# ultralytics/yolov5

Measured on NVIDIA H100. Metric: images/sec @640 (forward + NMS), higher is better.
Workload: dtype bf16

## Files before the change

### include/y5b200.h

```cpp
#ifndef Y5B200_H
#define Y5B200_H
#include <stdint.h>

#if defined(__GNUC__)
#define Y5_API __attribute__((visibility("default")))
#else
#define Y5_API
#endif

#ifdef __cplusplus
extern "C" {
#endif

#define Y5_F16 0
#define Y5_BF16 1
#define Y5_F32 2
#define Y5_U8 3

#define Y5_E_INVALID (-1)
#define Y5_E_UNSUPPORTED (-2)
#define Y5_E_DRIVER (-3)

#define Y5_ACT_NONE 0
#define Y5_ACT_SILU 1
// ... 25 lines not shown
    int64_t in_n_stride;
    int32_t a_mode;
    int32_t reserved;
} y5_conv_desc;

int y5_conv_pick(int32_t in_c, int32_t out_c, int64_t m_rows, int32_t* block_k, int32_t* block_n);

typedef struct y5_conv_plan y5_conv_plan;
int y5_conv_plan_create(const y5_conv_desc* desc, y5_conv_plan** plan);
int y5_conv_plan_run(const y5_conv_plan* plan, void* stream);
void y5_conv_plan_destroy(y5_conv_plan* plan);
struct y5_conv_plan_info {
    int32_t a_mode;
    int32_t tw, th;
    int32_t block_k, block_n, mt;
    int32_t cluster;
    int32_t patch_pw;
    int32_t b_grouped;
    int32_t staged;
    int32_t opt;
    int32_t epi;
    int32_t a_stages, b_stages;
    int32_t grid;
};
int y5_conv_plan_info(const y5_conv_plan* plan, struct y5_conv_plan_info* info);
int y5_conv_bn_silu_fwd(const y5_conv_desc* desc, void* stream);
int y5_conv_direct_fwd(const y5_conv_desc* desc, void* stream);

typedef struct y5_detect_desc {
    const void* in;
    int32_t in_pitch;
    int32_t batch, ny, nx, in_c;
    const void* weight;
    const float* bias;
    void* raw;
    void* z;
    int32_t z_rows, z_row0;
    int32_t na, no, nc;
    float stride;
    float anchor_wh[8];
    int32_t dtype;
    int32_t block_k;
} y5_detect_desc;
typedef struct y5_detect_plan y5_detect_plan;
int y5_detect_plan_create(const y5_detect_desc* desc, y5_detect_plan** plan);
int y5_detect_plan_run(const y5_detect_plan* plan, void* stream);
// ... 305 lines not shown
```

### yolov5_b200/_lib.py

```python
from __future__ import annotations

import ctypes as C
import os

import torch

_HERE = os.path.dirname(os.path.abspath(__file__))
LIB_PATH = os.environ.get("Y5B200_LIB") or os.path.join(_HERE, "liby5b200.so")

Y5_F16, Y5_BF16, Y5_F32, Y5_U8 = 0, 1, 2, 3
ACT_NONE, ACT_SILU = 0, 1

_DTYPE = {torch.float16: Y5_F16, torch.bfloat16: Y5_BF16, torch.float32: Y5_F32, torch.uint8: Y5_U8}


def dtype_code(dt: torch.dtype) -> int:
    try:
        return _DTYPE[dt]
    except KeyError:
        raise TypeError(f"y5b200: unsupported dtype {dt}") from None


class ConvDesc(C.Structure):
    _fields_ = [
# ... 9 lines not shown
        ("a_mode", C.c_int32), ("reserved", C.c_int32),
    ]


class DetectDesc(C.Structure):
    _fields_ = [
        ("inp", C.c_void_p), ("in_pitch", C.c_int32),
        ("batch", C.c_int32), ("ny", C.c_int32), ("nx", C.c_int32), ("in_c", C.c_int32),
        ("weight", C.c_void_p), ("bias", C.c_void_p),
        ("raw", C.c_void_p), ("z", C.c_void_p),
        ("z_rows", C.c_int32), ("z_row0", C.c_int32),
        ("na", C.c_int32), ("no", C.c_int32), ("nc", C.c_int32),
        ("stride", C.c_float), ("anchor_wh", C.c_float * 8),
        ("dtype", C.c_int32), ("block_k", C.c_int32),
    ]


class PlanInfo(C.Structure):
    _fields_ = [
        ("a_mode", C.c_int32), ("tw", C.c_int32), ("th", C.c_int32),
        ("block_k", C.c_int32), ("block_n", C.c_int32), ("mt", C.c_int32), ("cluster", C.c_int32),
        ("patch_pw", C.c_int32), ("b_grouped", C.c_int32), ("staged", C.c_int32), ("opt", C.c_int32), ("epi", C.c_int32),
        ("a_stages", C.c_int32), ("b_stages", C.c_int32), ("grid", C.c_int32),
    ]

    def as_dict(self) -> dict:
        return {f: getattr(self, f) for f, _ in self._fields_}


class NmsParams(C.Structure):
    _fields_ = [
        ("batch", C.c_int32), ("n_rows", C.c_int32), ("no", C.c_int32), ("nc", C.c_int32), ("nm", C.c_int32),
        ("dtype", C.c_int32), ("conf_thres", C.c_float), ("iou_thres", C.c_float),
        ("multi_label", C.c_int32), ("agnostic", C.c_int32), ("max_det", C.c_int32), ("max_nms", C.c_int32),
        ("max_wh", C.c_float), ("classes", C.c_void_p), ("n_classes", C.c_int32),
    ]


class LossParams(C.Structure):
    _fields_ = [
        ("nl", C.c_int32), ("batch", C.c_int32), ("na", C.c_int32), ("no", C.c_int32), ("nc", C.c_int32),
        ("ny", C.c_int32 * 5), ("nx", C.c_int32 * 5),
        ("dtype", C.c_int32), ("nt", C.c_int32),
        ("anchor_t", C.c_float), ("box_gain", C.c_float), ("obj_gain", C.c_float), ("cls_gain", C.c_float),
        ("cls_pw", C.c_float), ("obj_pw", C.c_float), ("cp", C.c_float), ("cn", C.c_float),
        ("balance", C.c_float * 5), ("grad_scale", C.c_float),
# ... 213 lines not shown
```

### yolov5_b200/csrc/common.cuh

```cuda
#pragma once
#include <cuda.h>
#include <cuda_bf16.h>
#include <cuda_fp16.h>
#include <cuda_runtime.h>
#include <stdint.h>
#include <stdio.h>

namespace y5 {

__device__ __forceinline__ uint32_t smem_u32(const void* p) { return static_cast<uint32_t>(__cvta_generic_to_shared(p)); }

__device__ __forceinline__ bool elect_one() {
    uint32_t pred = 0;
    asm volatile(
        "{\n\t.reg .pred P;\n\t"
        "elect.sync _|P, 0xffffffff;\n\t"
        "selp.b32 %0, 1, 0, P;\n\t}"
        : "=r"(pred));
    return pred != 0;
}

__device__ __forceinline__ void mbar_init(uint64_t* bar, uint32_t count) {
    asm volatile("mbarrier.init.shared::cta.b64 [%0], %1;" ::"r"(smem_u32(bar)), "r"(count) : "memory");
}
// ... 105 lines not shown
    return (((8u * row_bytes) >> 4) & 0x3FFFu) | (layout << 30);
}
__device__ __forceinline__ uint32_t gmma_desc_lo(uint32_t saddr) { return ((saddr >> 4) & 0x3FFFu) | (1u << 16); }
__device__ __forceinline__ uint64_t gmma_desc(uint32_t lo, uint32_t hi) { return (static_cast<uint64_t>(hi) << 32) | lo; }

__device__ __forceinline__ void wgmma_fence() { asm volatile("wgmma.fence.sync.aligned;" ::: "memory"); }
__device__ __forceinline__ void wgmma_commit() { asm volatile("wgmma.commit_group.sync.aligned;" ::: "memory"); }
template <int N>
__device__ __forceinline__ void wgmma_wait() { asm volatile("wgmma.wait_group.sync.aligned %0;" ::"n"(N) : "memory"); }
template <int N>
__device__ __forceinline__ void fence_regs(float (&d)[N]) {
#pragma unroll
    for (int i = 0; i < N; ++i) asm volatile("" : "+f"(d[i])::"memory");
}

template <uint32_t R>
__device__ __forceinline__ void setmaxnreg_dec() { asm volatile("setmaxnreg.dec.sync.aligned.u32 %0;" ::"n"(R)); }
template <uint32_t R>
__device__ __forceinline__ void setmaxnreg_inc() { asm volatile("setmaxnreg.inc.sync.aligned.u32 %0;" ::"n"(R)); }

__device__ __forceinline__ void griddep_wait() { asm volatile("griddepcontrol.wait;" ::: "memory"); }
__device__ __forceinline__ void griddep_launch_dependents() { asm volatile("griddepcontrol.launch_dependents;" ::: "memory"); }

__device__ __forceinline__ void named_bar_sync(uint32_t id, uint32_t nthreads) {
    asm volatile("bar.sync %0, %1;" ::"r"(id), "r"(nthreads) : "memory");
}

#ifndef Y5_SILU_EXACT
__device__ __forceinline__ float silu_f(float x) {
    const float h = 0.5f * x;
    float t;
    asm("tanh.approx.f32 %0, %1;" : "=f"(t) : "f"(h));
    return fmaf(h, t, h);
}
__device__ __forceinline__ float silu_from_half(float h) {
    float t;
    asm("tanh.approx.f32 %0, %1;" : "=f"(t) : "f"(h));
    return fmaf(h, t, h);
}
#else
__device__ __forceinline__ float silu_f(float x) { return __fdividef(x, 1.0f + __expf(-x)); }
__device__ __forceinline__ float silu_from_half(float h) { return silu_f(2.0f * h); }
#endif
__device__ __forceinline__ float silu_tail(float x) {
    float e;
    asm("ex2.approx.f32 %0, %1;" : "=f"(e) : "f"(1.44269504088896341f * x));
// ... 31 lines not shown
```

### yolov5_b200/csrc/conv_gemm.cu

```cuda
#include <cstdio>
#include <cstdlib>
#include <cstring>
#include <mutex>
#include <type_traits>

#include "../../include/y5b200.h"
#include "common.cuh"
#include "host_util.h"
#include "wgmma.cuh"

namespace y5 {

constexpr int kBlockM = 128;
constexpr int kConsumers = 2;
constexpr int kConsumerThreads = 128 * kConsumers;
constexpr int kThreads = 128 + kConsumerThreads;
constexpr int kMaxStages = 8;
constexpr int kHeadN = 128;

enum AMode { A_LINEAR = 0, A_IM2COL = 1, A_PATCH = 2 };

struct ConvParams {
    int M, N;
    int num_m_tiles;
    int num_m_super, num_n_tiles;
    int kh, kw, c_chunks;
    int block_k;
    int a_mode;
    int Ho, Wo, HoWo, stride, pad_h, pad_w;
    int tw, th, tiles_x, tiles_y;
    int b_grouped;
    int patch_pw;
    int cluster_n;
    uint32_t stg_bytes;
    uint32_t b_sub_bytes;
    float rcp_per_img, rcp_tiles_x, rcp_HoWo, rcp_Wo;
    int a_stages, b_stages;
    uint32_t a_sub_bytes, a_stage_bytes, b_stage_bytes;
    int is_bf16, act;
    const float* bias;
    int bias_n;
    void* out;
    int out_pitch;
    const void* res;
    int res_pitch;
    void* raw;
    void* z;
    int na, no, nc, nx, z_rows, z_row0;
    float det_stride;
    float anchor_wh[8];
};

struct SmemLayout {
    uint32_t off_a, off_b, off_out, off_bias, off_bars, total;
};

__host__ __device__ inline SmemLayout smem_layout(int epi, int no, int bias_n, int a_stages, int b_stages, uint32_t a_bytes,
                                                   uint32_t b_bytes, uint32_t stg_bytes) {
    SmemLayout L;
    uint32_t o = 0;
    L.off_a = o;
    o += a_stages * a_bytes;
    L.off_b = o;
    o += b_stages * b_bytes;
    o = (o + 1023) & ~1023u;
    L.off_out = o;
    if (epi == 1) o += 4 * ((kBlockM * no * 2 + 1023) & ~1023u);
    else o += stg_bytes;
    L.off_bias = o;
    o += ((bias_n + 3) & ~3) * 4;
    o = (o + 7) & ~7u;
    L.off_bars = o;
    o += 4 * kMaxStages * 8;
    L.total = o;
    return L;
}

__device__ __forceinline__ int fdiv(int n, int d, float rd) {
    if (n >= (1 << 23)) return n / d;
    int q = __float2int_rz(__int2float_rz(n) * rd);
    const int r = n - q * d;
    if (r >= d) ++q;
    else if (r < 0) --q;
    return q;
}

template <int BLOCK_N, int MT, int KS, bool BF16>
__device__ __forceinline__ void mma_batch(float (&acc)[MT][BLOCK_N / 2], uint32_t a_lo, uint32_t a_sub16, uint32_t a_hi, uint32_t b_lo,
                                          uint32_t b_hi, uint32_t scale_first) {
    wgmma_fence();
#pragma unroll
    for (int k = 0; k < KS; ++k)
#pragma unroll
        for (int mi = 0; mi < MT; ++mi)
            Wgmma<BLOCK_N>::template run<BF16, 0, 0>(acc[mi], gmma_desc(a_lo + mi * a_sub16 + 2 * k, a_hi), gmma_desc(b_lo + 2 * k, b_hi),
                                                     k == 0 ? scale_first : 1u);
    wgmma_commit();
}

template <int BLOCK_N, int EPI, int MT, bool OPT, bool BF16>
__global__ void __launch_bounds__(kThreads, 1)
conv_gemm_kernel(const __grid_constant__ CUtensorMap tmA, const __grid_constant__ CUtensorMap tmB, const ConvParams p) {
    static_assert(MT * BLOCK_N <= 256, "accumulators: at most 128 fp32 registers per consumer thread");
    constexpr int kAcc = BLOCK_N / 2;

    extern __shared__ __align__(1024) uint8_t smem_raw[];
    uint8_t* smem = reinterpret_cast<uint8_t*>((reinterpret_cast<uintptr_t>(smem_raw) + 1023) & ~uintptr_t(1023));
    const SmemLayout L = smem_layout(EPI, p.no, p.bias_n, p.a_stages, p.b_stages, p.a_stage_bytes, p.b_stage_bytes, p.stg_bytes);
    uint8_t* sA = smem + L.off_a;
    uint8_t* sB = smem + L.off_b;
    float* sBias = reinterpret_cast<float*>(smem + L.off_bias);
    uint64_t* a_full = reinterpret_cast<uint64_t*>(smem + L.off_bars);
    uint64_t* a_empty = a_full + kMaxStages;
    uint64_t* b_full = a_empty + kMaxStages;
    uint64_t* b_empty = b_full + kMaxStages;

    const int warp = threadIdx.x >> 5;
    const int lane = threadIdx.x & 31;
    const int csize = OPT ? static_cast<int>(cluster_nctarank()) : 1;
    const uint32_t crank = OPT ? cluster_ctarank() : 0u;

    if (threadIdx.x == 0) {
        tma_prefetch_desc(&tmA);
        tma_prefetch_desc(&tmB);
        for (int s = 0; s < kMaxStages; ++s) {
            mbar_init(&a_full[s], 1);
            mbar_init(&a_empty[s], kConsumers);
            mbar_init(&b_full[s], 1);
            mbar_init(&b_empty[s], kConsumers * csize);
        }
        fence_barrier_init();
    }
    if (threadIdx.x >= 128)
        for (int i = threadIdx.x - 128; i < p.bias_n; i += kConsumerThreads) {
            const float b = i < p.N ? __ldg(p.bias + i) : 0.0f;
            sBias[i] = (EPI == 0 && p.act) ? 0.5f * b : b;
        }
    __syncthreads();
    if (csize > 1) cluster_sync_all();
    griddep_wait();
    griddep_launch_dependents();

    const int nn = p.num_n_tiles;
    const int num_tiles = ((p.num_m_super + csize - 1) / csize) * nn;
    const int tile0 = blockIdx.x / csize, tile_step = gridDim.x / csize;
    const uint32_t row_bytes = p.block_k * 2;
    const bool patch = p.a_mode == A_PATCH;
    const bool wide = OPT && p.patch_pw > 0;
    const int grp = wide ? p.kh * p.kw : (patch ? p.kh : 1);
    const int num_groups = wide ? p.c_chunks : (patch ? p.c_chunks * p.kw : p.kh * p.kw * p.c_chunks);

    if (warp < 4) {
        setmaxnreg_dec<56>();
    }
    if (warp == 0) {
        int as = 0, bs = 0;
        uint32_t aph = 0, bph = 0;
        for (int tile = tile0; tile < num_tiles; tile += tile_step) {
            const int ms = (tile / nn) * csize + static_cast<int>(crank);
            const int n0 = (tile - (tile / nn) * nn) * BLOCK_N;
            int img[MT], y0[MT], x0[MT];
#pragma unroll
            for (int mi = 0; mi < MT; ++mi) {
                const int mt = ms * MT + mi;
                img[mi] = y0[mi] = x0[mi] = 0;
                if (p.a_mode == A_IM2COL) {
                    const int m0 = mt * kBlockM;
                    img[mi] = fdiv(m0, p.HoWo, p.rcp_HoWo);
                    const int rem = m0 - img[mi] * p.HoWo;
                    const int oy = fdiv(rem, p.Wo, p.rcp_Wo);
                    y0[mi] = oy * p.stride - p.pad_h;
                    x0[mi] = (rem - oy * p.Wo) * p.stride - p.pad_w;
                } else if (patch) {
                    const int per_img = p.tiles_x * p.tiles_y;
                    img[mi] = fdiv(mt, per_img, p.rcp_per_img);
                    const int rem = mt - img[mi] * per_img;
                    const int ty = fdiv(rem, p.tiles_x, p.rcp_tiles_x);
                    y0[mi] = ty * p.th - p.pad_h;
                    x0[mi] = (rem - ty * p.tiles_x) * p.tw - p.pad_w;
                }
// ... 25 lines not shown
                        if (stage_first) mbar_arrive_expect_tx(&b_full[bs], p.b_stage_bytes);
                        uint8_t* b_dst = sB + bs * p.b_stage_bytes + (p.b_grouped ? j * p.b_sub_bytes : 0u);
                        if (csize == 1) tma_load_2d(&tmB, &b_full[bs], b_dst, kb * p.block_k, n0);
                        else {
                            const int slice_rows = BLOCK_N / csize;
                            tma_load_2d_mcast(&tmB, &b_full[bs], b_dst + crank * slice_rows * row_bytes, kb * p.block_k,
                                              n0 + static_cast<int>(crank) * slice_rows, static_cast<uint16_t>((1u << csize) - 1u));
                        }
                    }
                    __syncwarp();
                    if (stage_last && ++bs == p.b_stages) { bs = 0; bph ^= 1; }
                }
            };
            if (wide) {
                for (int cc = 0; cc < p.c_chunks; ++cc) issue_group(cc, 0, 0);
            } else if (patch) {
                for (int cc = 0; cc < p.c_chunks; ++cc)
                    for (int s = 0; s < p.kw; ++s) issue_group(cc, s, 0);
            } else {
                for (int r = 0; r < p.kh; ++r)
                    for (int s = 0; s < p.kw; ++s)
                        for (int cc = 0; cc < p.c_chunks; ++cc) issue_group(cc, s, r);
            }
        }
    } else if (warp >= 4) {
    setmaxnreg_inc<224>();
    const int wg = (warp >> 2) - 1;
    const int ct = threadIdx.x - 128;
    const int wrow = wg * 64 + (warp & 3) * 16 + (lane >> 2);
    const int ccol = 2 * (lane & 3);
    const bool signal = (threadIdx.x & 127) == 0;
    constexpr bool bf16 = BF16;
    const uint32_t dhi = gmma_desc_hi(row_bytes);
    const uint32_t a_hi = wide ? (dhi & ~0x3FFFu) | (((static_cast<uint32_t>(p.patch_pw) * row_bytes) >> 4) & 0x3FFFu) : dhi;
    const uint32_t a_base = gmma_desc_lo(smem_u32(sA) + (wide ? wg * 8 * p.patch_pw : wg * 64) * row_bytes), b_base = gmma_desc_lo(smem_u32(sB));
    const uint32_t row16 = row_bytes >> 4;
    const uint32_t a_stage16 = p.a_stage_bytes >> 4, b_stage16 = p.b_stage_bytes >> 4, a_sub16 = p.a_sub_bytes >> 4;
    const uint32_t b_sub16 = p.b_sub_bytes >> 4;
    const uint32_t a_shift16 = patch ? (p.tw * row_bytes) >> 4 : 0;
    const int k_steps = p.block_k / 16;
    const int per_img = p.tiles_x * p.tiles_y;
    const int tw_shift = patch ? __ffs(p.tw) - 1 : 0;
    int as = 0, bs = 0, head_set = 0;
    uint32_t aph = 0, bph = 0;
    float acc[MT][kAcc];
#pragma unroll
    for (int mi = 0; mi < MT; ++mi)
#pragma unroll
        for (int i = 0; i < kAcc; ++i) acc[mi][i] = 0.0f;

    int pend_as = 0, pend_bs = 0;
    bool pend_a_last = false, pend_b_last = false;
    auto release_pending = [&]() {
        if (!signal) return;
        if (pend_b_last) {
            if (csize == 1) mbar_arrive(&b_empty[pend_bs]);
            else
                for (int r = 0; r < csize; ++r) mbar_arrive_cluster(mapa_u32(&b_empty[pend_bs], static_cast<uint32_t>(r)));
        }
        if (pend_a_last) mbar_arrive(&a_empty[pend_as]);
    };

    for (int tile = tile0; tile < num_tiles; tile += tile_step) {
        const int ms = (tile / nn) * csize + static_cast<int>(crank);
        const int nt = tile - (tile / nn) * nn;
        const int n0 = nt * BLOCK_N;
        for (int g = 0; g < num_groups; ++g) {
            mbar_wait(&a_full[as], aph);
            const uint32_t a_stage_lo = a_base + as * a_stage16;
            uint32_t a_lo = a_stage_lo;
            for (int j = 0; j < grp; ++j) {
                if (wide) {
                    const int tr = j / p.kw, ts = j - tr * p.kw;
                    a_lo = a_stage_lo + (tr * p.patch_pw + ts) * row16;
                }
                const bool stage_first = !p.b_grouped || j == 0, stage_last = !p.b_grouped || j == grp - 1;
                if (stage_first) mbar_wait(&b_full[bs], bph);
                const uint32_t b_lo = b_base + bs * b_stage16 + (p.b_grouped ? j * b_sub16 : 0u);
                const uint32_t scale_first = (g | j) != 0 ? 1u : 0u;
#pragma unroll
                for (int mi = 0; mi < MT; ++mi) fence_regs(acc[mi]);
                switch (k_steps) {
                    case 4: mma_batch<BLOCK_N, MT, 4, BF16>(acc, a_lo, a_sub16, a_hi, b_lo, dhi, scale_first); break;
                    case 2: mma_batch<BLOCK_N, MT, 2, BF16>(acc, a_lo, a_sub16, a_hi, b_lo, dhi, scale_first); break;
                    default: mma_batch<BLOCK_N, MT, 1, BF16>(acc, a_lo, a_sub16, a_hi, b_lo, dhi, scale_first); break;
                }
                wgmma_wait<1>();
#pragma unroll
                for (int mi = 0; mi < MT; ++mi) fence_regs(acc[mi]);
                if (g | j) release_pending();
                pend_as = as;
                pend_a_last = j == grp - 1;
                pend_bs = bs;
                pend_b_last = stage_last;
                if (stage_last && ++bs == p.b_stages) { bs = 0; bph ^= 1; }
                a_lo += a_shift16;
            }
            if (++as == p.a_stages) { as = 0; aph ^= 1; }
        }
        wgmma_wait<0>();
#pragma unroll
        for (int mi = 0; mi < MT; ++mi) fence_regs(acc[mi]);
        release_pending();

        if (EPI == 0) {
            const bool staged = OPT && p.stg_bytes != 0;
            const uint32_t stg_pitch = BLOCK_N * 2 + 16;
            uint8_t* stg = smem + L.off_out + wg * 64 * stg_pitch;
            auto pixel_of = [&](int mt, int row) -> long long {
                if (patch) {
                    const int img = fdiv(mt, per_img, p.rcp_per_img);
                    const int rem = mt - img * per_img;
                    const int tyi = fdiv(rem, p.tiles_x, p.rcp_tiles_x);
                    const int oy = tyi * p.th + (row >> tw_shift), ox = (rem - tyi * p.tiles_x) * p.tw + (row & ((1 << tw_shift) - 1));
                    return (mt < p.num_m_tiles && oy < p.Ho && ox < p.Wo) ? static_cast<long long>(img) * p.HoWo + oy * p.Wo + ox : -1;
                }
                const long long m = static_cast<long long>(mt) * kBlockM + row;
                return m < p.M ? m : -1;
            };
            constexpr float kTail = BF16 ? 8.0f : 4.0f;
            constexpr int kRows = 2 * MT, kWords = (OPT ? 128 : 256) / BLOCK_N;
            constexpr int kBatch = kWords < 1 ? 1 : (kWords < kRows ? kWords : kRows);
            const bool has_res = p.res != nullptr;
#pragma unroll
            for (int q0 = 0; q0 < kRows; q0 += kBatch) {
                uint32_t rv[kBatch][BLOCK_N / 8];
                long long gp[kBatch];
#pragma unroll
                for (int q = 0; q < kBatch; ++q) gp[q] = pixel_of(ms * MT + (q0 + q) / 2, wrow + 8 * ((q0 + q) & 1));
                if (has_res) {
#pragma unroll
                    for (int q = 0; q < kBatch; ++q) {
                        const uint16_t* rp = reinterpret_cast<const uint16_t*>(p.res) + (gp[q] < 0 ? 0 : gp[q] * p.res_pitch) + n0 + ccol;
#pragma unroll
                        for (int j = 0; j < BLOCK_N / 8; ++j)
                            rv[q][j] = (gp[q] >= 0 && n0 + 8 * j < p.N) ? *reinterpret_cast<const uint32_t*>(rp + 8 * j) : 0u;
                    }
                }
#pragma unroll
                for (int q = 0; q < kBatch; ++q) {
                    const int mi = (q0 + q) / 2, h = (q0 + q) & 1;
                    const int mt = ms * MT + mi;
                    const int row = wrow + 8 * h;
                    const long long gpix = gp[q];
                    if (gpix >= 0 || staged) {
                        uint16_t* op = reinterpret_cast<uint16_t*>(p.out) + gpix * p.out_pitch + n0 + ccol;
                        uint8_t* sp = stg + (row - wg * 64) * stg_pitch + ccol * 2;
                        float hmin = 0.0f;
                        auto row_half = [&](auto tail_pass) {
                            constexpr bool TAIL = decltype(tail_pass)::value;
#pragma unroll
                            for (int j = 0; j < BLOCK_N / 8; ++j) {
                                if (n0 + 8 * j >= p.N) continue;
                                const float2 b = *reinterpret_cast<const float2*>(sBias + n0 + 8 * j + ccol);
                                const float a0 = acc[mi][4 * j + 2 * h], a1 = acc[mi][4 * j + 2 * h + 1];
                                float f0, f1;
                                if (p.act) {
                                    const float h0 = fmaf(a0, 0.5f, b.x), h1 = fmaf(a1, 0.5f, b.y);
                                    f0 = silu_from_half(h0);
                                    f1 = silu_from_half(h1);
                                    if (TAIL) {
                                        if (h0 < -0.5f * kTail) f0 = silu_tail(2.0f * h0);
                                        if (h1 < -0.5f * kTail) f1 = silu_tail(2.0f * h1);
                                    } else {
                                        hmin = fminf(hmin, fminf(h0, h1));
                                    }
                                } else {
                                    f0 = a0 + b.x;
                                    f1 = a1 + b.y;
                                }
                                if (has_res && gpix >= 0) {
                                    const float2 t = unpack2(rv[q][j], bf16);
                                    f0 += t.x;
                                    f1 += t.y;
                                }
                                if (staged) *reinterpret_cast<uint32_t*>(sp + 16 * j) = pack2(f0, f1, bf16);
                                else *reinterpret_cast<uint32_t*>(op + 8 * j) = pack2(f0, f1, bf16);
                            }
                        };
                        row_half(std::false_type{});
                        if (p.act && __any_sync(__activemask(), hmin < -0.5f * kTail)) row_half(std::true_type{});
                    }
                    if (staged && h == 1) {
                        named_bar_sync(2 + wg, 128);
                        constexpr int kSeg = BLOCK_N / 8;
                        for (int i = threadIdx.x & 127; i < 64 * kSeg; i += 128) {
                            const int lrow = i / kSeg, c = i - lrow * kSeg;
                            const long long gp = pixel_of(mt, wg * 64 + lrow);
                            if (gp >= 0 && n0 + 8 * c < p.N)
                                *reinterpret_cast<uint4*>(reinterpret_cast<uint16_t*>(p.out) + gp * p.out_pitch + n0 + 8 * c) =
                                    *reinterpret_cast<const uint4*>(stg + lrow * stg_pitch + c * 16);
                        }
                        named_bar_sync(2 + wg, 128);
                    }
                }
            }
        } else {
            const uint32_t blk = (kBlockM * p.no * 2 + 1023) & ~1023u;
            const int set = head_set;
            head_set ^= 1;
            uint16_t* stage_raw = reinterpret_cast<uint16_t*>(smem + L.off_out + (2 * set) * blk);
            uint16_t* stage_z = reinterpret_cast<uint16_t*>(smem + L.off_out + (2 * set + 1) * blk);
            const int no = p.no;
            const int a = nt;
            const float aw = p.anchor_wh[a * 2], ah = p.anchor_wh[a * 2 + 1];
            const int m0 = ms * kBlockM;
            const int rows_here = min(kBlockM, p.M - m0);
#pragma unroll
            for (int h = 0; h < 2; ++h) {
                const int row = wrow + 8 * h;
                const int m = m0 + row;
                int gx = 0, gy = 0;
                if (m < p.M) { const int pix = m - fdiv(m, p.HoWo, p.rcp_HoWo) * p.HoWo; gy = fdiv(pix, p.nx, p.rcp_Wo); gx = pix - gy * p.nx; }
                const float fgx = static_cast<float>(gx) - 0.5f, fgy = static_cast<float>(gy) - 0.5f;
#pragma unroll
                for (int j = 0; j < BLOCK_N / 8; ++j) {
#pragma unroll
// ... 84 lines not shown
}

void pick_tile(int out_c, int64_t m_tiles, int* block_n, int* mt) {
    const int64_t sms = sm_count();
    if (out_c <= 32) { *block_n = 32; *mt = 4; return; }
    if (out_c <= 64) { *block_n = 64; *mt = 2; return; }
    if (out_c <= 128) {
        *block_n = 128;
        *mt = ((m_tiles + 1) / 2) >= sms ? 2 : 1;
        return;
    }
    const int64_t tiles256 = m_tiles * ((out_c + 255) / 256);
    *block_n = (tiles256 >= 2 * sms && (out_c % 256 == 0 || out_c > 384)) ? 256 : 128;
    *mt = 1;
}

int pick_block_n(int out_c, int64_t m_rows) {
    int bn, mt;
    pick_tile(out_c, m_rows > 0 ? (m_rows + kBlockM - 1) / kBlockM : 1, &bn, &mt);
    return bn;
}

template <int BN, int EPI, int MT, bool OPT>
cudaError_t launch_conv(const CUtensorMap& a, const CUtensorMap& b, const ConvParams& p, int grid, int cluster, uint32_t smem,
                        cudaStream_t st) {
    auto* kernel = p.is_bf16 ? conv_gemm_kernel<BN, EPI, MT, OPT, true> : conv_gemm_kernel<BN, EPI, MT, OPT, false>;
    const cudaError_t attr_err = ensure_dyn_smem(reinterpret_cast<const void*>(kernel), 227 * 1024);
    if (attr_err != cudaSuccess) return attr_err;
    count_launch();
    if (cluster == 1) return launch_pdl(kernel, dim3(grid), dim3(kThreads), smem, st, a, b, p);
    static const bool pdl = [] { const char* e = getenv("Y5_PDL"); return !(e && e[0] == '0'); }();
    cudaLaunchConfig_t cfg{};
    cfg.gridDim = dim3(grid);
    cfg.blockDim = dim3(kThreads);
    cfg.dynamicSmemBytes = smem;
    cfg.stream = st;
    cudaLaunchAttribute attr[2];
    attr[0].id = cudaLaunchAttributeClusterDimension;
    attr[0].val.clusterDim.x = cluster;
    attr[0].val.clusterDim.y = 1;
    attr[0].val.clusterDim.z = 1;
    attr[1].id = cudaLaunchAttributeProgrammaticStreamSerialization;
    attr[1].val.programmaticStreamSerializationAllowed = 1;
    cfg.attrs = attr;
    cfg.numAttrs = pdl ? 2 : 1;
    return cudaLaunchKernelEx(&cfg, kernel, a, b, p);
}

struct PlanCommon {
    CUtensorMap tmA, tmB;
    ConvParams p;
    int block_n, epi, mt, grid, cluster;
    uint32_t smem_bytes;
};

int finish_plan(PlanCommon& pc, int block_n, int epi, int mt, int cluster = 1) {
    ConvParams& p = pc.p;
    p.cluster_n = cluster;
    p.a_stage_bytes = mt * p.a_sub_bytes;
    if (p.patch_pw > 0) p.a_stage_bytes = static_cast<uint32_t>(p.th + p.kh - 1) * p.patch_pw * p.block_k * 2;
    p.num_m_super = (p.num_m_tiles + mt - 1) / mt;
    p.num_n_tiles = epi == 1 ? p.na : (p.N + block_n - 1) / block_n;
    p.bias_n = p.num_n_tiles * block_n;
    const uint32_t budget = 225 * 1024 - 1024;
    const bool patch = p.a_mode == A_PATCH;
    int a_st = 0, b_st = 0;
    if (!patch) {
        for (int s = kMaxStages; s >= 2; --s)
            if (smem_layout(epi, p.no, p.bias_n, s, s, p.a_stage_bytes, p.b_stage_bytes, p.stg_bytes).total <= budget) { a_st = b_st = s; break; }
    } else {
        const int b_min = p.b_grouped ? 2 : 3, b_max = p.b_grouped ? 4 : kMaxStages;
        for (int a = 3; a >= 2 && !a_st; --a)
            for (int b = b_max; b >= b_min; --b)
                if (smem_layout(epi, p.no, p.bias_n, a, b, p.a_stage_bytes, p.b_stage_bytes, p.stg_bytes).total <= budget) { a_st = a; b_st = b; break; }
    }
    if (a_st < 2 || b_st < 2) return set_error(Y5_E_UNSUPPORTED, "conv tile does not fit shared memory (block_n %d a %u b %u)", block_n,
                                                p.a_stage_bytes, p.b_stage_bytes);
    p.a_stages = a_st;
    p.b_stages = b_st;
    pc.smem_bytes = smem_layout(epi, p.no, p.bias_n, a_st, b_st, p.a_stage_bytes, p.b_stage_bytes, p.stg_bytes).total + 1024;
    pc.block_n = block_n;
    pc.epi = epi;
    pc.mt = mt;
    pc.cluster = cluster;
    const long long tiles = static_cast<long long>((p.num_m_super + cluster - 1) / cluster) * p.num_n_tiles;
    const int max_clusters = sm_count() / cluster;
    pc.grid = static_cast<int>(tiles < max_clusters ? tiles : max_clusters) * cluster;
    return 0;
}

bool plan_opt(const PlanCommon& pc) { return pc.cluster > 1 || pc.p.patch_pw > 0 || pc.p.stg_bytes > 0; }

int run_plan(const PlanCommon& pc, cudaStream_t st) {
    cudaError_t e = cudaErrorInvalidValue;
    const int key = (plan_opt(pc) ? 100000 : 0) + pc.epi * 10000 + pc.block_n * 10 + pc.mt;
    switch (key) {
        case 324: e = launch_conv<32, 0, 4, false>(pc.tmA, pc.tmB, pc.p, pc.grid, pc.cluster, pc.smem_bytes, st); break;
        case 642: e = launch_conv<64, 0, 2, false>(pc.tmA, pc.tmB, pc.p, pc.grid, pc.cluster, pc.smem_bytes, st); break;
        case 1281: e = launch_conv<128, 0, 1, false>(pc.tmA, pc.tmB, pc.p, pc.grid, pc.cluster, pc.smem_bytes, st); break;
        case 1282: e = launch_conv<128, 0, 2, false>(pc.tmA, pc.tmB, pc.p, pc.grid, pc.cluster, pc.smem_bytes, st); break;
        case 2561: e = launch_conv<256, 0, 1, false>(pc.tmA, pc.tmB, pc.p, pc.grid, pc.cluster, pc.smem_bytes, st); break;
        case 11281: e = launch_conv<kHeadN, 1, 1, false>(pc.tmA, pc.tmB, pc.p, pc.grid, pc.cluster, pc.smem_bytes, st); break;
        case 100324: e = launch_conv<32, 0, 4, true>(pc.tmA, pc.tmB, pc.p, pc.grid, pc.cluster, pc.smem_bytes, st); break;
        case 100642: e = launch_conv<64, 0, 2, true>(pc.tmA, pc.tmB, pc.p, pc.grid, pc.cluster, pc.smem_bytes, st); break;
        case 101281: e = launch_conv<128, 0, 1, true>(pc.tmA, pc.tmB, pc.p, pc.grid, pc.cluster, pc.smem_bytes, st); break;
        case 101282: e = launch_conv<128, 0, 2, true>(pc.tmA, pc.tmB, pc.p, pc.grid, pc.cluster, pc.smem_bytes, st); break;
        case 102561: e = launch_conv<256, 0, 1, true>(pc.tmA, pc.tmB, pc.p, pc.grid, pc.cluster, pc.smem_bytes, st); break;
        default: return set_error(Y5_E_UNSUPPORTED, "conv: no kernel for block_n %d mt %d epi %d", pc.block_n, pc.mt, pc.epi);
    }
    if (e != cudaSuccess) return set_error(int(e), "conv_gemm launch failed: %s", cudaGetErrorString(e));
    return 0;
}

bool aligned16(const void* p) { return (reinterpret_cast<uintptr_t>(p) & 15) == 0; }

struct Geo {
    int kh, kw, pad_h, pad_w, Ho, Wo;
    long long xs, ys, ns;
};
Geo geometry(const y5_conv_desc* d) {
    Geo g;
    g.kh = d->ksize;
    g.kw = d->kw ? d->kw : d->ksize;
    g.pad_h = d->pad;
    g.pad_w = d->kw ? d->pad_w : d->pad;
    g.xs = d->in_x_stride ? d->in_x_stride : d->in_pitch;
    g.ys = d->in_y_stride ? d->in_y_stride : static_cast<long long>(d->in_w) * g.xs;
    g.ns = d->in_n_stride ? d->in_n_stride : static_cast<long long>(d->in_h) * g.ys;
    g.Ho = (d->in_h + 2 * g.pad_h - g.kh) / d->stride + 1;
    g.Wo = (d->in_w + 2 * g.pad_w - g.kw) / d->stride + 1;
    return g;
}

}

struct y5_conv_plan {
    PlanCommon pc;
};
struct y5_detect_plan {
    PlanCommon pc;
};

extern "C" Y5_API int y5_conv_pick(int32_t in_c, int32_t out_c, int64_t m_rows, int32_t* block_k, int32_t* block_n) {
    if (in_c <= 0 || out_c <= 0) return set_error(Y5_E_INVALID, "y5_conv_pick: non-positive channel count");
    if (block_k) *block_k = pick_block_k(in_c);
    if (block_n) *block_n = pick_block_n(out_c, m_rows);
    return 0;
}

static int validate_conv(const y5_conv_desc* d) {
    if (!d || !d->in || !d->weight || !d->bias || !d->out) return set_error(Y5_E_INVALID, "conv: null pointer");
    if (d->dtype != Y5_F16 && d->dtype != Y5_BF16) return set_error(Y5_E_UNSUPPORTED, "conv: dtype must be fp16/bf16");
    if (d->batch <= 0 || d->in_h <= 0 || d->in_w <= 0 || d->in_c <= 0 || d->out_c <= 0)
        return set_error(Y5_E_INVALID, "conv: non-positive dimension");
// ... 108 lines not shown
            p.b_grouped = 1;
            p.b_stage_bytes = g.kh * p.b_sub_bytes;
        }
        p.tiles_x = (g.Wo + p.tw - 1) / p.tw;
        p.tiles_y = (g.Ho + p.th - 1) / p.th;
        p.rcp_tiles_x = 1.0f / static_cast<float>(p.tiles_x);
        p.rcp_per_img = 1.0f / static_cast<float>(p.tiles_x * p.tiles_y);
        p.num_m_tiles = d->batch * p.tiles_x * p.tiles_y;
        p.a_sub_bytes = p.patch_pw ? 8 * row_bytes : (p.th + g.kh - 1) * p.tw * row_bytes;
        cuuint64_t dims[4] = {(cuuint64_t)d->in_c, (cuuint64_t)d->in_w, (cuuint64_t)d->in_h, (cuuint64_t)d->batch};
        cuuint64_t str[3] = {(cuuint64_t)g.xs * 2, (cuuint64_t)g.ys * 2, (cuuint64_t)g.ns * 2};
        cuuint32_t box[4] = {(cuuint32_t)bk, (cuuint32_t)(p.patch_pw ? p.patch_pw : p.tw), (cuuint32_t)(p.th + g.kh - 1), 1};
        e = encode_tiled(&pc.tmA, d->dtype, d->in, 4, dims, str, box, sw, "A patch");
    }
    if (e) { delete plan; return e; }
    const uint64_t ktot = static_cast<uint64_t>(p.kh) * p.kw * p.c_chunks * bk;
    {
        cuuint64_t dims[2] = {ktot, (cuuint64_t)d->out_c};
        cuuint64_t str[1] = {ktot * 2};
        cuuint32_t box[2] = {(cuuint32_t)bk, (cuuint32_t)(bn / cl_sel)};
        e = encode_tiled(&pc.tmB, d->dtype, d->weight, 2, dims, str, box, sw, "B");
    }
    if (e) { delete plan; return e; }
    p.stg_bytes = ((d->reserved & 8) && !(d->reserved & 16)) ? static_cast<uint32_t>(kConsumers * 64 * (bn * 2 + 16)) : 0u;
    int e2 = finish_plan(pc, bn, 0, mt_sel, cl_sel);
    if (e2 && p.stg_bytes) {
        p.stg_bytes = 0;
        e2 = finish_plan(pc, bn, 0, mt_sel, cl_sel);
    }
    if (e2) { delete plan; return e2; }
    *out = plan;
    return 0;
}

extern "C" Y5_API int y5_conv_plan_run(const y5_conv_plan* plan, void* stream) {
    if (!plan) return set_error(Y5_E_INVALID, "conv: null plan");
    return run_plan(plan->pc, static_cast<cudaStream_t>(stream));
}
extern "C" Y5_API void y5_conv_plan_destroy(y5_conv_plan* plan) { delete plan; }

extern "C" Y5_API int y5_conv_plan_info(const y5_conv_plan* plan, struct y5_conv_plan_info* out) {
    if (!plan || !out) return set_error(Y5_E_INVALID, "conv: null plan/info");
    const PlanCommon& pc = plan->pc;
    const ConvParams& p = pc.p;
    out->a_mode = p.a_mode;
    out->tw = p.tw;
    out->th = p.th;
    out->block_k = p.block_k;
    out->block_n = pc.block_n;
    out->mt = pc.mt;
    out->cluster = pc.cluster;
    out->patch_pw = p.patch_pw;
    out->b_grouped = p.b_grouped;
    out->staged = p.stg_bytes > 0;
    out->opt = plan_opt(pc);
    out->epi = pc.epi;
    out->a_stages = p.a_stages;
    out->b_stages = p.b_stages;
    out->grid = pc.grid;
    return 0;
}

extern "C" Y5_API int y5_conv_bn_silu_fwd(const y5_conv_desc* d, void* stream) {
    y5_conv_plan* plan = nullptr;
    if (int e = y5_conv_plan_create(d, &plan)) return e;
    const int e = y5_conv_plan_run(plan, stream);
    y5_conv_plan_destroy(plan);
    return e;
}

extern "C" Y5_API int y5_conv_direct_fwd(const y5_conv_desc* d, void* stream) {
    if (int e = validate_conv(d)) return e;
    const Geo g = geometry(d);
    const int bk = d->block_k ? d->block_k : pick_block_k(d->in_c);
    const int cin_pad = (d->in_c + bk - 1) / bk * bk;
    const long long total = static_cast<long long>(d->batch) * g.Ho * g.Wo * d->out_c;
    const int threads = 256;
// ... 78 lines not shown
```

Baseline: 2987.

## Add TMA-based epilogue with swizzled smem staging and TMA residual prefetch

Adds a TMA epilogue path for non-optimized conv GEMM plans. The producer warp prefetches residual tiles into swizzled shared memory through TMA, and consumers write their results there before issuing TMA stores. New mbarriers coordinate reuse of the staging buffer across tiles. The aim is to replace scattered per-thread global stores and residual loads with bulk async copies that overlap with the next tile's mainloop, at the cost of extra shared memory and more synchronisation.

Result: faster. 3204 (median of 6 runs) (+7.2%).

```diff
diff --git a/include/y5b200.h b/include/y5b200.h
--- a/include/y5b200.h
+++ b/include/y5b200.h
@@ -71,6 +71,7 @@
     int32_t epi;
     int32_t a_stages, b_stages;
     int32_t grid;
+    int32_t tma_epi;
 };
 int y5_conv_plan_info(const y5_conv_plan* plan, struct y5_conv_plan_info* info);
 int y5_conv_bn_silu_fwd(const y5_conv_desc* desc, void* stream);
diff --git a/yolov5_b200/_lib.py b/yolov5_b200/_lib.py
--- a/yolov5_b200/_lib.py
+++ b/yolov5_b200/_lib.py
@@ -55,6 +55,7 @@
         ("block_k", C.c_int32), ("block_n", C.c_int32), ("mt", C.c_int32), ("cluster", C.c_int32),
         ("patch_pw", C.c_int32), ("b_grouped", C.c_int32), ("staged", C.c_int32), ("opt", C.c_int32), ("epi", C.c_int32),
         ("a_stages", C.c_int32), ("b_stages", C.c_int32), ("grid", C.c_int32),
+        ("tma_epi", C.c_int32),
     ]
 
     def as_dict(self) -> dict:
diff --git a/yolov5_b200/csrc/common.cuh b/yolov5_b200/csrc/common.cuh
--- a/yolov5_b200/csrc/common.cuh
+++ b/yolov5_b200/csrc/common.cuh
@@ -151,6 +151,15 @@
 __device__ __forceinline__ void griddep_wait() { asm volatile("griddepcontrol.wait;" ::: "memory"); }
 __device__ __forceinline__ void griddep_launch_dependents() { asm volatile("griddepcontrol.launch_dependents;" ::: "memory"); }
 
+__device__ __forceinline__ uint32_t ld_shared_u32(uint32_t addr) {
+    uint32_t v;
+    asm volatile("ld.shared.b32 %0, [%1];" : "=r"(v) : "r"(addr) : "memory");
+    return v;
+}
+__device__ __forceinline__ void st_shared_u32(uint32_t addr, uint32_t v) {
+    asm volatile("st.shared.b32 [%0], %1;" ::"r"(addr), "r"(v) : "memory");
+}
+
 __device__ __forceinline__ void named_bar_sync(uint32_t id, uint32_t nthreads) {
     asm volatile("bar.sync %0, %1;" ::"r"(id), "r"(nthreads) : "memory");
 }
diff --git a/yolov5_b200/csrc/conv_gemm.cu b/yolov5_b200/csrc/conv_gemm.cu
--- a/yolov5_b200/csrc/conv_gemm.cu
+++ b/yolov5_b200/csrc/conv_gemm.cu
@@ -33,6 +33,7 @@
     int patch_pw;
     int cluster_n;
     uint32_t stg_bytes;
+    int tma_epi;
     uint32_t b_sub_bytes;
     float rcp_per_img, rcp_tiles_x, rcp_HoWo, rcp_Wo;
     int a_stages, b_stages;
@@ -71,7 +72,7 @@
     o += ((bias_n + 3) & ~3) * 4;
     o = (o + 7) & ~7u;
     L.off_bars = o;
-    o += 4 * kMaxStages * 8;
+    o += (4 * kMaxStages + 2) * 8;
     L.total = o;
     return L;
 }
@@ -85,6 +86,26 @@
     return q;
 }
 
+template <int BLOCK_N>
+struct EpiBox {
+    static constexpr int kRB = BLOCK_N * 2 < 128 ? BLOCK_N * 2 : 128;
+    static constexpr int kCols = kRB / 2;
+    static constexpr int kNB = BLOCK_N / kCols;
+    static constexpr uint32_t kBytes = 64u * kRB;
+};
+struct EpiOrigin {
+    int x, y, img;
+};
+__device__ __forceinline__ EpiOrigin epi_origin(const ConvParams& p, int mt, int wg) {
+    if (p.a_mode != A_PATCH) return {0, mt * kBlockM + 64 * wg, 0};
+    const int per_img = p.tiles_x * p.tiles_y;
+    const int img = fdiv(mt, per_img, p.rcp_per_img);
+    const int rem = mt - img * per_img;
+    const int ty = fdiv(rem, p.tiles_x, p.rcp_tiles_x);
+    const int x = (rem - ty * p.tiles_x) * p.tw, y = ty * p.th;
+    return p.tw > 64 ? EpiOrigin{x + 64 * wg, y, img} : EpiOrigin{x, y + wg * (64 / p.tw), img};
+}
+
 template <int BLOCK_N, int MT, int KS, bool BF16>
 __device__ __forceinline__ void mma_batch(float (&acc)[MT][BLOCK_N / 2], uint32_t a_lo, uint32_t a_sub16, uint32_t a_hi, uint32_t b_lo,
                                           uint32_t b_hi, uint32_t scale_first) {
@@ -100,9 +121,12 @@
 
 template <int BLOCK_N, int EPI, int MT, bool OPT, bool BF16>
 __global__ void __launch_bounds__(kThreads, 1)
-conv_gemm_kernel(const __grid_constant__ CUtensorMap tmA, const __grid_constant__ CUtensorMap tmB, const ConvParams p) {
+conv_gemm_kernel(const __grid_constant__ CUtensorMap tmA, const __grid_constant__ CUtensorMap tmB, const __grid_constant__ CUtensorMap tmO,
+                 const __grid_constant__ CUtensorMap tmR, const ConvParams p) {
     static_assert(MT * BLOCK_N <= 256, "accumulators: at most 128 fp32 registers per consumer thread");
     constexpr int kAcc = BLOCK_N / 2;
+    using Box = EpiBox<BLOCK_N>;
+    const bool tma_epi = EPI == 0 && !OPT && p.tma_epi;
 
     extern __shared__ __align__(1024) uint8_t smem_raw[];
     uint8_t* smem = reinterpret_cast<uint8_t*>((reinterpret_cast<uintptr_t>(smem_raw) + 1023) & ~uintptr_t(1023));
@@ -114,6 +138,9 @@
     uint64_t* a_empty = a_full + kMaxStages;
     uint64_t* b_full = a_empty + kMaxStages;
     uint64_t* b_empty = b_full + kMaxStages;
+    uint64_t* res_full = b_empty + kMaxStages;
+    uint64_t* stg_free = res_full + 1;
+    uint8_t* stg = smem + L.off_out;
 
     const int warp = threadIdx.x >> 5;
     const int lane = threadIdx.x & 31;
@@ -129,6 +156,12 @@
             mbar_init(&b_full[s], 1);
             mbar_init(&b_empty[s], kConsumers * csize);
         }
+        mbar_init(res_full, 1);
+        mbar_init(stg_free, kConsumers);
+        if (tma_epi) {
+            tma_prefetch_desc(&tmO);
+            if (p.res) tma_prefetch_desc(&tmR);
+        }
         fence_barrier_init();
     }
     if (threadIdx.x >= 128)
@@ -155,7 +188,7 @@
     }
     if (warp == 0) {
         int as = 0, bs = 0;
-        uint32_t aph = 0, bph = 0;
+        uint32_t aph = 0, bph = 0, sph = 0;
         for (int tile = tile0; tile < num_tiles; tile += tile_step) {
             const int ms = (tile / nn) * csize + static_cast<int>(crank);
             const int n0 = (tile - (tile / nn) * nn) * BLOCK_N;
@@ -227,6 +260,28 @@
                     for (int s = 0; s < p.kw; ++s)
                         for (int cc = 0; cc < p.c_chunks; ++cc) issue_group(cc, s, r);
             }
+            if (tma_epi) {
+                mbar_wait(stg_free, sph ^ 1);
+                if (elect_one()) {
+                    if (p.res) {
+                        mbar_arrive_expect_tx(res_full, p.stg_bytes);
+#pragma unroll 1
+                        for (int i = 0; i < kConsumers * MT; ++i) {
+                            const EpiOrigin o = epi_origin(p, ms * MT + i % MT, i / MT);
+#pragma unroll
+                            for (int b = 0; b < Box::kNB; ++b) {
+                                uint8_t* dst = stg + (i * Box::kNB + b) * Box::kBytes;
+                                if (patch) tma_load_4d(&tmR, res_full, dst, n0 + b * Box::kCols, o.x, o.y, o.img);
+                                else tma_load_2d(&tmR, res_full, dst, n0 + b * Box::kCols, o.y);
+                            }
+                        }
+                    } else {
+                        mbar_arrive(res_full);
+                    }
+                }
+                __syncwarp();
+                sph ^= 1;
+            }
         }
     } else if (warp >= 4) {
     setmaxnreg_inc<224>();
@@ -247,7 +302,7 @@
     const int per_img = p.tiles_x * p.tiles_y;
     const int tw_shift = patch ? __ffs(p.tw) - 1 : 0;
     int as = 0, bs = 0, head_set = 0;
-    uint32_t aph = 0, bph = 0;
+    uint32_t aph = 0, bph = 0, rph = 0;
     float acc[MT][kAcc];
 #pragma unroll
     for (int mi = 0; mi < MT; ++mi)
@@ -294,6 +349,10 @@
 #pragma unroll
                 for (int mi = 0; mi < MT; ++mi) fence_regs(acc[mi]);
                 if (g | j) release_pending();
+                else if (tma_epi && signal && tile != tile0) {
+                    tma_store_wait_read0();
+                    mbar_arrive(stg_free);
+                }
                 pend_as = as;
                 pend_a_last = j == grp - 1;
                 pend_bs = bs;
@@ -311,7 +370,14 @@
         if (EPI == 0) {
             const bool staged = OPT && p.stg_bytes != 0;
             const uint32_t stg_pitch = BLOCK_N * 2 + 16;
-            uint8_t* stg = smem + L.off_out + wg * 64 * stg_pitch;
+            uint8_t* stg_wg = stg + wg * 64 * stg_pitch;
+            constexpr int kChunks = Box::kRB / 16;
+            uint32_t stg_row = smem_u32(stg) + wg * MT * Box::kNB * Box::kBytes + (wrow - wg * 64) * Box::kRB + ccol * 2;
+            uint32_t stg_swz = ((((wrow - wg * 64) * Box::kRB) >> 7) & (kChunks - 1)) << 4;
+            asm volatile("" : "+r"(stg_row), "+r"(stg_swz));
+            auto stg_word = [&](int mi, int h, int j) -> uint32_t {
+                return stg_row + (mi * Box::kNB + j / kChunks) * Box::kBytes + h * 8 * Box::kRB + (((j % kChunks) << 4) ^ stg_swz);
+            };
             auto pixel_of = [&](int mt, int row) -> long long {
                 if (patch) {
                     const int img = fdiv(mt, per_img, p.rcp_per_img);
@@ -327,77 +393,110 @@
             constexpr int kRows = 2 * MT, kWords = (OPT ? 128 : 256) / BLOCK_N;
             constexpr int kBatch = kWords < 1 ? 1 : (kWords < kRows ? kWords : kRows);
             const bool has_res = p.res != nullptr;
-#pragma unroll
-            for (int q0 = 0; q0 < kRows; q0 += kBatch) {
-                uint32_t rv[kBatch][BLOCK_N / 8];
-                long long gp[kBatch];
-#pragma unroll
-                for (int q = 0; q < kBatch; ++q) gp[q] = pixel_of(ms * MT + (q0 + q) / 2, wrow + 8 * ((q0 + q) & 1));
-                if (has_res) {
+            if (tma_epi) {
+                mbar_wait(res_full, rph);
+                rph ^= 1;
+            }
+            auto rows = [&](auto tma_path) {
+                constexpr bool TMA = decltype(tma_path)::value;
+#pragma unroll
+                for (int q0 = 0; q0 < kRows; q0 += kBatch) {
+                    uint32_t rv[kBatch][BLOCK_N / 8];
+                    long long gp[kBatch];
+#pragma unroll
+                    for (int q = 0; q < kBatch; ++q) gp[q] = TMA ? 0 : pixel_of(ms * MT + (q0 + q) / 2, wrow + 8 * ((q0 + q) & 1));
+                    if (has_res && TMA) {
+#pragma unroll
+                        for (int q = 0; q < kBatch; ++q)
+#pragma unroll
+                            for (int j = 0; j < BLOCK_N / 8; ++j) rv[q][j] = ld_shared_u32(stg_word((q0 + q) / 2, (q0 + q) & 1, j));
+                    } else if (has_res) {
+#pragma unroll
+                        for (int q = 0; q < kBatch; ++q) {
+                            const uint16_t* rp = reinterpret_cast<const uint16_t*>(p.res) + (gp[q] < 0 ? 0 : gp[q] * p.res_pitch) + n0 + ccol;
+#pragma unroll
+                            for (int j = 0; j < BLOCK_N / 8; ++j)
+                                rv[q][j] = (gp[q] >= 0 && n0 + 8 * j < p.N) ? *reinterpret_cast<const uint32_t*>(rp + 8 * j) : 0u;
+                        }
+                    }
 #pragma unroll
                     for (int q = 0; q < kBatch; ++q) {
-                        const uint16_t* rp = reinterpret_cast<const uint16_t*>(p.res) + (gp[q] < 0 ? 0 : gp[q] * p.res_pitch) + n0 + ccol;
-#pragma unroll
-                        for (int j = 0; j < BLOCK_N / 8; ++j)
-                            rv[q][j] = (gp[q] >= 0 && n0 + 8 * j < p.N) ? *reinterpret_cast<const uint32_t*>(rp + 8 * j) : 0u;
+                        const int mi = (q0 + q) / 2, h = (q0 + q) & 1;
+                        const int mt = ms * MT + mi;
+                        const int row = wrow + 8 * h;
+                        const long long gpix = gp[q];
+                        if (gpix >= 0 || staged) {
+                            uint16_t* op = reinterpret_cast<uint16_t*>(p.out) + gpix * p.out_pitch + n0 + ccol;
+                            uint8_t* sp = stg_wg + (row - wg * 64) * stg_pitch + ccol * 2;
+                            float hmin = 0.0f;
+                            auto row_half = [&](auto tail_pass) {
+                                constexpr bool TAIL = decltype(tail_pass)::value;
+#pragma unroll
+                                for (int j = 0; j < BLOCK_N / 8; ++j) {
+                                    if (n0 + 8 * j >= p.N) continue;
+                                    const float2 b = *reinterpret_cast<const float2*>(sBias + n0 + 8 * j + ccol);
+                                    const float a0 = acc[mi][4 * j + 2 * h], a1 = acc[mi][4 * j + 2 * h + 1];
+                                    float f0, f1;
+                                    if (p.act) {
+                                        const float h0 = fmaf(a0, 0.5f, b.x), h1 = fmaf(a1, 0.5f, b.y);
+                                        f0 = silu_from_half(h0);
+                                        f1 = silu_from_half(h1);
+                                        if (TAIL) {
+                                            if (h0 < -0.5f * kTail) f0 = silu_tail(2.0f * h0);
+                                            if (h1 < -0.5f * kTail) f1 = silu_tail(2.0f * h1);
+                                        } else {
+                                            hmin = fminf(hmin, fminf(h0, h1));
+                                        }
+                                    } else {
+                                        f0 = a0 + b.x;
+                                        f1 = a1 + b.y;
+                                    }
+                                    if (has_res && gpix >= 0) {
+                                        const float2 t = unpack2(rv[q][j], bf16);
+                                        f0 += t.x;
+                                        f1 += t.y;
+                                    }
+                                    if (TMA) st_shared_u32(stg_word(mi, h, j), pack2(f0, f1, bf16));
+                                    else if (staged) *reinterpret_cast<uint32_t*>(sp + 16 * j) = pack2(f0, f1, bf16);
+                                    else *reinterpret_cast<uint32_t*>(op + 8 * j) = pack2(f0, f1, bf16);
+                                }
+                            };
+                            row_half(std::false_type{});
+                            if (p.act && __any_sync(__activemask(), hmin < -0.5f * kTail)) row_half(std::true_type{});
+                        }
+                        if (staged && h == 1) {
+                            named_bar_sync(2 + wg, 128);
+                            constexpr int kSeg = BLOCK_N / 8;
+                            for (int i = threadIdx.x & 127; i < 64 * kSeg; i += 128) {
+                                const int lrow = i / kSeg, c = i - lrow * kSeg;
+                                const long long gp = pixel_of(mt, wg * 64 + lrow);
+                                if (gp >= 0 && n0 + 8 * c < p.N)
+                                    *reinterpret_cast<uint4*>(reinterpret_cast<uint16_t*>(p.out) + gp * p.out_pitch + n0 + 8 * c) =
+                                        *reinterpret_cast<const uint4*>(stg_wg + lrow * stg_pitch + c * 16);
+                            }
+                            named_bar_sync(2 + wg, 128);
+                        }
                     }
                 }
-#pragma unroll
-                for (int q = 0; q < kBatch; ++q) {
-                    const int mi = (q0 + q) / 2, h = (q0 + q) & 1;
-                    const int mt = ms * MT + mi;
-                    const int row = wrow + 8 * h;
-                    const long long gpix = gp[q];
-                    if (gpix >= 0 || staged) {
-                        uint16_t* op = reinterpret_cast<uint16_t*>(p.out) + gpix * p.out_pitch + n0 + ccol;
-                        uint8_t* sp = stg + (row - wg * 64) * stg_pitch + ccol * 2;
-                        float hmin = 0.0f;
-                        auto row_half = [&](auto tail_pass) {
-                            constexpr bool TAIL = decltype(tail_pass)::value;
-#pragma unroll
-                            for (int j = 0; j < BLOCK_N / 8; ++j) {
-                                if (n0 + 8 * j >= p.N) continue;
-                                const float2 b = *reinterpret_cast<const float2*>(sBias + n0 + 8 * j + ccol);
-                                const float a0 = acc[mi][4 * j + 2 * h], a1 = acc[mi][4 * j + 2 * h + 1];
-                                float f0, f1;
-                                if (p.act) {
-                                    const float h0 = fmaf(a0, 0.5f, b.x), h1 = fmaf(a1, 0.5f, b.y);
-                                    f0 = silu_from_half(h0);
-                                    f1 = silu_from_half(h1);
-                                    if (TAIL) {
-                                        if (h0 < -0.5f * kTail) f0 = silu_tail(2.0f * h0);
-                                        if (h1 < -0.5f * kTail) f1 = silu_tail(2.0f * h1);
-                                    } else {
-                                        hmin = fminf(hmin, fminf(h0, h1));
-                                    }
-                                } else {
-                                    f0 = a0 + b.x;
-                                    f1 = a1 + b.y;
-                                }
-                                if (has_res && gpix >= 0) {
-                                    const float2 t = unpack2(rv[q][j], bf16);
-                                    f0 += t.x;
-                                    f1 += t.y;
-                                }
-                                if (staged) *reinterpret_cast<uint32_t*>(sp + 16 * j) = pack2(f0, f1, bf16);
-                                else *reinterpret_cast<uint32_t*>(op + 8 * j) = pack2(f0, f1, bf16);
-                            }
-                        };
-                        row_half(std::false_type{});
-                        if (p.act && __any_sync(__activemask(), hmin < -0.5f * kTail)) row_half(std::true_type{});
+            };
+            if (tma_epi) rows(std::true_type{});
+            else rows(std::false_type{});
+            if (tma_epi) {
+                fence_proxy_async_smem();
+                named_bar_sync(2 + wg, 128);
+                if (signal) {
+#pragma unroll 1
+                    for (int mi = 0; mi < MT; ++mi) {
+                        const EpiOrigin o = epi_origin(p, ms * MT + mi, wg);
+#pragma unroll
+                        for (int b = 0; b < Box::kNB; ++b) {
+                            const uint8_t* src = stg + ((wg * MT + mi) * Box::kNB + b) * Box::kBytes;
+                            if (patch) tma_store_4d(&tmO, src, n0 + b * Box::kCols, o.x, o.y, o.img);
+                            else tma_store_2d(&tmO, src, n0 + b * Box::kCols, o.y);
+                        }
                     }
-                    if (staged && h == 1) {
-                        named_bar_sync(2 + wg, 128);
-                        constexpr int kSeg = BLOCK_N / 8;
-                        for (int i = threadIdx.x & 127; i < 64 * kSeg; i += 128) {
-                            const int lrow = i / kSeg, c = i - lrow * kSeg;
-                            const long long gp = pixel_of(mt, wg * 64 + lrow);
-                            if (gp >= 0 && n0 + 8 * c < p.N)
-                                *reinterpret_cast<uint4*>(reinterpret_cast<uint16_t*>(p.out) + gp * p.out_pitch + n0 + 8 * c) =
-                                    *reinterpret_cast<const uint4*>(stg + lrow * stg_pitch + c * 16);
-                        }
-                        named_bar_sync(2 + wg, 128);
-                    }
+                    tma_store_commit();
+                    if (tile + tile_step >= num_tiles) tma_store_wait_all();
                 }
             }
         } else {
@@ -528,13 +627,13 @@
 }
 
 template <int BN, int EPI, int MT, bool OPT>
-cudaError_t launch_conv(const CUtensorMap& a, const CUtensorMap& b, const ConvParams& p, int grid, int cluster, uint32_t smem,
-                        cudaStream_t st) {
+cudaError_t launch_conv(const CUtensorMap& a, const CUtensorMap& b, const CUtensorMap& o, const CUtensorMap& r, const ConvParams& p,
+                        int grid, int cluster, uint32_t smem, cudaStream_t st) {
     auto* kernel = p.is_bf16 ? conv_gemm_kernel<BN, EPI, MT, OPT, true> : conv_gemm_kernel<BN, EPI, MT, OPT, false>;
     const cudaError_t attr_err = ensure_dyn_smem(reinterpret_cast<const void*>(kernel), 227 * 1024);
     if (attr_err != cudaSuccess) return attr_err;
     count_launch();
-    if (cluster == 1) return launch_pdl(kernel, dim3(grid), dim3(kThreads), smem, st, a, b, p);
+    if (cluster == 1) return launch_pdl(kernel, dim3(grid), dim3(kThreads), smem, st, a, b, o, r, p);
     static const bool pdl = [] { const char* e = getenv("Y5_PDL"); return !(e && e[0] == '0'); }();
     cudaLaunchConfig_t cfg{};
     cfg.gridDim = dim3(grid);
@@ -550,11 +649,12 @@
     attr[1].val.programmaticStreamSerializationAllowed = 1;
     cfg.attrs = attr;
     cfg.numAttrs = pdl ? 2 : 1;
-    return cudaLaunchKernelEx(&cfg, kernel, a, b, p);
+    return cudaLaunchKernelEx(&cfg, kernel, a, b, o, r, p);
 }
 
 struct PlanCommon {
     CUtensorMap tmA, tmB;
+    CUtensorMap tmO, tmR;
     ConvParams p;
     int block_n, epi, mt, grid, cluster;
     uint32_t smem_bytes;
@@ -595,23 +695,24 @@
     return 0;
 }
 
-bool plan_opt(const PlanCommon& pc) { return pc.cluster > 1 || pc.p.patch_pw > 0 || pc.p.stg_bytes > 0; }
+bool plan_staged(const PlanCommon& pc) { return pc.p.stg_bytes > 0 && !pc.p.tma_epi; }
+bool plan_opt(const PlanCommon& pc) { return pc.cluster > 1 || pc.p.patch_pw > 0 || plan_staged(pc); }
 
 int run_plan(const PlanCommon& pc, cudaStream_t st) {
     cudaError_t e = cudaErrorInvalidValue;
     const int key = (plan_opt(pc) ? 100000 : 0) + pc.epi * 10000 + pc.block_n * 10 + pc.mt;
     switch (key) {
-        case 324: e = launch_conv<32, 0, 4, false>(pc.tmA, pc.tmB, pc.p, pc.grid, pc.cluster, pc.smem_bytes, st); break;
-        case 642: e = launch_conv<64, 0, 2, false>(pc.tmA, pc.tmB, pc.p, pc.grid, pc.cluster, pc.smem_bytes, st); break;
-        case 1281: e = launch_conv<128, 0, 1, false>(pc.tmA, pc.tmB, pc.p, pc.grid, pc.cluster, pc.smem_bytes, st); break;
-        case 1282: e = launch_conv<128, 0, 2, false>(pc.tmA, pc.tmB, pc.p, pc.grid, pc.cluster, pc.smem_bytes, st); break;
-        case 2561: e = launch_conv<256, 0, 1, false>(pc.tmA, pc.tmB, pc.p, pc.grid, pc.cluster, pc.smem_bytes, st); break;
-        case 11281: e = launch_conv<kHeadN, 1, 1, false>(pc.tmA, pc.tmB, pc.p, pc.grid, pc.cluster, pc.smem_bytes, st); break;
-        case 100324: e = launch_conv<32, 0, 4, true>(pc.tmA, pc.tmB, pc.p, pc.grid, pc.cluster, pc.smem_bytes, st); break;
-        case 100642: e = launch_conv<64, 0, 2, true>(pc.tmA, pc.tmB, pc.p, pc.grid, pc.cluster, pc.smem_bytes, st); break;
-        case 101281: e = launch_conv<128, 0, 1, true>(pc.tmA, pc.tmB, pc.p, pc.grid, pc.cluster, pc.smem_bytes, st); break;
-        case 101282: e = launch_conv<128, 0, 2, true>(pc.tmA, pc.tmB, pc.p, pc.grid, pc.cluster, pc.smem_bytes, st); break;
-        case 102561: e = launch_conv<256, 0, 1, true>(pc.tmA, pc.tmB, pc.p, pc.grid, pc.cluster, pc.smem_bytes, st); break;
+        case 324: e = launch_conv<32, 0, 4, false>(pc.tmA, pc.tmB, pc.tmO, pc.tmR, pc.p, pc.grid, pc.cluster, pc.smem_bytes, st); break;
+        case 642: e = launch_conv<64, 0, 2, false>(pc.tmA, pc.tmB, pc.tmO, pc.tmR, pc.p, pc.grid, pc.cluster, pc.smem_bytes, st); break;
+        case 1281: e = launch_conv<128, 0, 1, false>(pc.tmA, pc.tmB, pc.tmO, pc.tmR, pc.p, pc.grid, pc.cluster, pc.smem_bytes, st); break;
+        case 1282: e = launch_conv<128, 0, 2, false>(pc.tmA, pc.tmB, pc.tmO, pc.tmR, pc.p, pc.grid, pc.cluster, pc.smem_bytes, st); break;
+        case 2561: e = launch_conv<256, 0, 1, false>(pc.tmA, pc.tmB, pc.tmO, pc.tmR, pc.p, pc.grid, pc.cluster, pc.smem_bytes, st); break;
+        case 11281: e = launch_conv<kHeadN, 1, 1, false>(pc.tmA, pc.tmB, pc.tmO, pc.tmR, pc.p, pc.grid, pc.cluster, pc.smem_bytes, st); break;
+        case 100324: e = launch_conv<32, 0, 4, true>(pc.tmA, pc.tmB, pc.tmO, pc.tmR, pc.p, pc.grid, pc.cluster, pc.smem_bytes, st); break;
+        case 100642: e = launch_conv<64, 0, 2, true>(pc.tmA, pc.tmB, pc.tmO, pc.tmR, pc.p, pc.grid, pc.cluster, pc.smem_bytes, st); break;
+        case 101281: e = launch_conv<128, 0, 1, true>(pc.tmA, pc.tmB, pc.tmO, pc.tmR, pc.p, pc.grid, pc.cluster, pc.smem_bytes, st); break;
+        case 101282: e = launch_conv<128, 0, 2, true>(pc.tmA, pc.tmB, pc.tmO, pc.tmR, pc.p, pc.grid, pc.cluster, pc.smem_bytes, st); break;
+        case 102561: e = launch_conv<256, 0, 1, true>(pc.tmA, pc.tmB, pc.tmO, pc.tmR, pc.p, pc.grid, pc.cluster, pc.smem_bytes, st); break;
         default: return set_error(Y5_E_UNSUPPORTED, "conv: no kernel for block_n %d mt %d epi %d", pc.block_n, pc.mt, pc.epi);
     }
     if (e != cudaSuccess) return set_error(int(e), "conv_gemm launch failed: %s", cudaGetErrorString(e));
@@ -636,6 +737,21 @@
     g.Ho = (d->in_h + 2 * g.pad_h - g.kh) / d->stride + 1;
     g.Wo = (d->in_w + 2 * g.pad_w - g.kw) / d->stride + 1;
     return g;
+}
+
+int encode_epi_map(CUtensorMap* map, int dtype, const void* base, int pitch, const ConvParams& p, int batch, int bn, const char* what) {
+    const int rb = bn * 2 < 128 ? bn * 2 : 128;
+    const cuuint64_t px = static_cast<cuuint64_t>(pitch) * 2;
+    if (p.a_mode == A_PATCH) {
+        cuuint64_t dims[4] = {(cuuint64_t)p.N, (cuuint64_t)p.Wo, (cuuint64_t)p.Ho, (cuuint64_t)batch};
+        cuuint64_t str[3] = {px, px * p.Wo, px * p.HoWo};
+        cuuint32_t box[4] = {(cuuint32_t)(rb / 2), (cuuint32_t)(p.tw < 64 ? p.tw : 64), (cuuint32_t)(p.tw < 64 ? 64 / p.tw : 1), 1};
+        return encode_tiled(map, dtype, base, 4, dims, str, box, swizzle_for_row_bytes(rb), what);
+    }
+    cuuint64_t dims[2] = {(cuuint64_t)p.N, (cuuint64_t)p.M};
+    cuuint64_t str[1] = {px};
+    cuuint32_t box[2] = {(cuuint32_t)(rb / 2), 64};
+    return encode_tiled(map, dtype, base, 2, dims, str, box, swizzle_for_row_bytes(rb), what);
 }
 
 }
@@ -790,10 +906,21 @@
         e = encode_tiled(&pc.tmB, d->dtype, d->weight, 2, dims, str, box, sw, "B");
     }
     if (e) { delete plan; return e; }
-    p.stg_bytes = ((d->reserved & 8) && !(d->reserved & 16)) ? static_cast<uint32_t>(kConsumers * 64 * (bn * 2 + 16)) : 0u;
+    const bool opt_modes = cl_sel > 1 || p.patch_pw > 0 || (d->reserved & 8);
+    const bool stages_first = p.a_mode == A_IM2COL && bn == 256;
+    if (!(d->reserved & 16) && !opt_modes && !stages_first) {
+        p.tma_epi = 1;
+        p.stg_bytes = static_cast<uint32_t>(mt_sel * bn * 256);
+        e = encode_epi_map(&pc.tmO, d->dtype, d->out, d->out_pitch, p, d->batch, bn, "output");
+        if (!e && d->residual) e = encode_epi_map(&pc.tmR, d->dtype, d->residual, d->res_pitch, p, d->batch, bn, "residual");
+        if (e) { delete plan; return e; }
+    } else if ((d->reserved & 8) && !(d->reserved & 16)) {
+        p.stg_bytes = static_cast<uint32_t>(kConsumers * 64 * (bn * 2 + 16));
+    }
     int e2 = finish_plan(pc, bn, 0, mt_sel, cl_sel);
     if (e2 && p.stg_bytes) {
         p.stg_bytes = 0;
+        p.tma_epi = 0;
         e2 = finish_plan(pc, bn, 0, mt_sel, cl_sel);
     }
     if (e2) { delete plan; return e2; }
@@ -820,7 +947,8 @@
     out->cluster = pc.cluster;
     out->patch_pw = p.patch_pw;
     out->b_grouped = p.b_grouped;
-    out->staged = p.stg_bytes > 0;
+    out->staged = plan_staged(pc);
+    out->tma_epi = p.tma_epi;
     out->opt = plan_opt(pc);
     out->epi = pc.epi;
     out->a_stages = p.a_stages;
```
